# jonnylaw/bayesian_dlms

Measured on AMD Instinct MI355X. Metric: Kalman filter+smooth series*timesteps/sec, higher is better.
Workload: dtype f64

## Files before the change

### bayesian_dlms_amd/csrc/dlm_engine.hip

```cpp
#include "../../include/dlm_engine.h"
#include <cstdlib>
#include "dlm_internal.h"

#include <rccl/rccl.h>

#include <cstdio>
#include <cstring>
#include <set>
#include <string>
#include <vector>

using dlm::KArgs;

struct dlm_engine {
  int device = 0;
  hipStream_t own_stream = nullptr;
  hipStream_t stream = nullptr;
  std::string err;
  const char* variant = "none";
  void* arena = nullptr;
  size_t arena_bytes = 0;
  hipEvent_t ev[3] = {nullptr, nullptr, nullptr};
  bool timed = false;
  dlm::SparseT* sp_dev = nullptr;
// ... 20 lines not shown
    long long f_stride = 0;
    unsigned generic = 0;
    int sparse_k = 0, spb_k = 0, spf_k = 0;
    bool have_spb = false, have_spf = false;
    std::vector<double> g_host, f_host;
  } an;
  bool an_touched = true;
  double* covws = nullptr;
  size_t covws_bytes = 0;
  unsigned char* route = nullptr;
  size_t route_bytes = 0;
  unsigned char* plainbuf = nullptr;
  size_t plainbuf_bytes = 0;
  void* sampws = nullptr;
  size_t sampws_bytes = 0;
  double* zws = nullptr;
  size_t zws_bytes = 0;
  hipStream_t rng_stream = nullptr;
  hipEvent_t rng_ev = nullptr;
  hipStream_t cov_stream = nullptr;
  hipEvent_t cov_ev[2] = {nullptr, nullptr};
  hipEvent_t rng_gate = nullptr;
  hipEvent_t cov_ev2 = nullptr;
  bool cov_busy = false, rng_busy = false;
  unsigned long long* counters = nullptr;
  unsigned long long* model_sum = nullptr;
  int* model_bad = nullptr;
  int* model_bad_dev = nullptr;
  bool model_sum_valid = false;
};

namespace {

int fail(dlm_engine* e, int code, const std::string& msg) {
  if (e) e->err = msg;
  return code;
}

int promise_broken(dlm_engine* e) {
  *e->model_bad = 0;
  e->an.valid = false;
  return fail(e, DLM_ERR_ARG, "DLM_OPT_MODEL_UNCHANGED was set, but F, G or the time grid differ from the model of the previous call (device checksum): the results of this call are invalid -- drop the flag when the model changes");
}

#define HIP_TRY(e, expr)                                                                    \
  do {                                                                                      \
// ... 356 lines not shown
  }
  return DLM_OK;
}
int mark_plain(dlm_engine* e, KArgs& k) {
  k.plain = nullptr;
  if (!(fast_shape_ok(k) && e->sparse_k > 0) || use_lane(k) || !k.y || k.g_index || k.dt || k.f_stride || k.v_tstride || k.w_tstride ||
      (k.flags & DLM_OPT_NO_STEADY)) return DLM_OK;
  if ((size_t)k.N > e->plainbuf_bytes) {
    if (e->plainbuf) { { const int rcd = drain_all(e); if (rcd) return rcd; } HIP_TRY(e, hipFree(e->plainbuf)); e->plainbuf = nullptr; e->plainbuf_bytes = 0; }
    HIP_TRY(e, hipMalloc((void**)&e->plainbuf, (size_t)k.N));
    e->plainbuf_bytes = (size_t)k.N;
  }
  HIP_TRY(e, dlm::launch_sparse16_count_gaps(k, e->plainbuf, e->stream));
  k.plain = e->plainbuf;
  return DLM_OK;
}
int ensure_cov_stream(dlm_engine* e) {
  if (!e->cov_stream) {
    int lo = 0, hi = 0;
    HIP_TRY(e, hipDeviceGetStreamPriorityRange(&lo, &hi));
    HIP_TRY(e, hipStreamCreateWithPriority(&e->cov_stream, hipStreamNonBlocking, hi));
    for (auto& ev : e->cov_ev) HIP_TRY(e, hipEventCreateWithFlags(&ev, hipEventDisableTiming));
    HIP_TRY(e, hipEventCreateWithFlags(&e->cov_ev2, hipEventDisableTiming));
  }
  return DLM_OK;
}
int start_sampler_normals(dlm_engine* e, const KArgs& k, dlm::SampTabs& tb, bool big, hipEvent_t gate);
int start_sampler_tables(dlm_engine* e, const KArgs& k, dlm::SampTabs& tb, bool big, const double* crec = nullptr, int crec_stride = 0, bool defer_normals = false) {
  const size_t need = big ? dlm::wave48_sampler_shared_ws_bytes(k) : dlm::sampler_shared_ws_bytes(k);
  if (need > e->sampws_bytes) {
    if (e->sampws) { { const int rcd = drain_all(e); if (rcd) return rcd; } HIP_TRY(e, hipFree(e->sampws)); e->sampws = nullptr; e->sampws_bytes = 0; }
    HIP_TRY(e, hipMalloc(&e->sampws, need));
    e->sampws_bytes = need;
  }
  int rc = ensure_route(e, (size_t)k.N);
  if (rc || (rc = ensure_cov_stream(e))) return rc;
  if (big) dlm::wave48_sampler_shared_carve(e->sampws, k, tb); else dlm::sampler_shared_carve(e->sampws, k, tb);
  HIP_TRY(e, hipEventRecord(e->cov_ev[0], e->stream));
  e->cov_busy = true;
  HIP_TRY(e, hipStreamWaitEvent(e->cov_stream, e->cov_ev[0], 0));
  tb.zstride = 0; tb.mc4 = nullptr; tb.marked = 0;
  if (big) HIP_TRY(e, dlm::launch_wave48_sampler_shared_tables(k, tb, e->cov_stream, e->cov_ev2));
  else if (crec) HIP_TRY(e, dlm::launch_sampler_shared_tables_from(k, e->sparse_k, e->sp_dev, tb, crec, crec_stride, e->cov_stream));
  else HIP_TRY(e, dlm::launch_sampler_shared_tables(k, e->sparse_k, e->sp_dev, tb, e->cov_stream));
  HIP_TRY(e, hipEventRecord(e->cov_ev[1], e->cov_stream));
  tb.z4 = nullptr;
// ... 24 lines not shown
int start_rts_tables(dlm_engine* e, const KArgs& k, dlm::RtsTabs& tb) {
  const size_t need = dlm::rts_shared_ws_bytes(k);
  if (need > e->sampws_bytes) {
    if (e->sampws) { { const int rcd = drain_all(e); if (rcd) return rcd; } HIP_TRY(e, hipFree(e->sampws)); e->sampws = nullptr; e->sampws_bytes = 0; }
    HIP_TRY(e, hipMalloc(&e->sampws, need));
    e->sampws_bytes = need;
  }
  const size_t cneed = sizeof(double) * dlm::covtabs_doubles(k.d, k.T);
  if (cneed > e->covws_bytes) {
    if (e->covws) { { const int rcd = drain_all(e); if (rcd) return rcd; } HIP_TRY(e, hipFree(e->covws)); e->covws = nullptr; e->covws_bytes = 0; }
    HIP_TRY(e, hipMalloc((void**)&e->covws, cneed));
    e->covws_bytes = cneed;
  }
  int rc = ensure_route(e, (size_t)k.N);
  if (rc || (rc = ensure_cov_stream(e))) return rc;
  dlm::rts_shared_carve(e->sampws, k, tb);
  dlm::CovTabs ctb{};
  dlm::covtabs_carve(e->covws, k.d, k.T, ctb);
  HIP_TRY(e, dlm::launch_rts_shared_mark(k, e->route, tb, e->stream));
  HIP_TRY(e, dlm::launch_rts_shared_cov(k, e->sparse_k, e->sp_dev, tb, ctb, e->stream));
  HIP_TRY(e, hipEventRecord(e->cov_ev[0], e->stream));
  e->cov_busy = true;
  HIP_TRY(e, hipStreamWaitEvent(e->cov_stream, e->cov_ev[0], 0));
  HIP_TRY(e, dlm::launch_rts_shared_tables(k, e->sparse_k, e->sp_dev, tb, e->cov_stream));
  HIP_TRY(e, hipEventRecord(e->cov_ev[1], e->cov_stream));
  return DLM_OK;
}
int ensure_shared(dlm_engine* e, const KArgs& k, dlm::CovTabs& tb, bool with_backward) {
  const size_t need = sizeof(double) * dlm::covtabs_doubles(k.d, k.T);
  if (need > e->covws_bytes) {
    if (e->covws) { { const int rcd = drain_all(e); if (rcd) return rcd; } HIP_TRY(e, hipFree(e->covws)); e->covws = nullptr; e->covws_bytes = 0; }
    HIP_TRY(e, hipMalloc((void**)&e->covws, need));
    e->covws_bytes = need;
  }
  int rc = ensure_route(e, (size_t)k.N);
  if (rc) return rc;
  rc = ensure_side(e, k);
  if (rc) return rc;
  if ((rc = ensure_cov_stream(e))) return rc;
  dlm::covtabs_carve(e->covws, k.d, k.T, tb);
  tb.eq = e->side + 2 * (size_t)k.N * ((size_t)k.T + 1);
  tb.mc = tb.sc = nullptr;
  if (with_backward) {
    const size_t one = 64 * (size_t)((k.N + 3) / 4) * ((size_t)k.T + 1);
    int rc2 = ensure_xplus_bytes(e, sizeof(double) * one);
    if (rc2) return rc2;
    tb.mc = e->xplus;
// ... 127 lines not shown

void dlm_engine_destroy(dlm_engine* e) {
  if (!e) return;
  (void)hipSetDevice(e->device);
  (void)drain_all(e);
  if (e->has_comm) ncclCommDestroy(e->comm);
  if (e->arena) (void)hipFree(e->arena);
  if (e->side) (void)hipFree(e->side);
  if (e->xplus) (void)hipFree(e->xplus);
  if (e->ystar) (void)hipFree(e->ystar);
  if (e->sp_dev) (void)hipFree(e->sp_dev);
  if (e->fws) (void)hipFree(e->fws);
  if (e->spb_dev) (void)hipFree(e->spb_dev);
  if (e->spf_dev) (void)hipFree(e->spf_dev);
  if (e->covws) (void)hipFree(e->covws);
  if (e->route) (void)hipFree(e->route);
  if (e->plainbuf) (void)hipFree(e->plainbuf);
  if (e->sampws) (void)hipFree(e->sampws);
  if (e->zws) (void)hipFree(e->zws);
  if (e->rng_ev) (void)hipEventDestroy(e->rng_ev);
  if (e->rng_stream) (void)hipStreamDestroy(e->rng_stream);
  for (auto& ev : e->cov_ev) if (ev) (void)hipEventDestroy(ev);
  if (e->cov_ev2) (void)hipEventDestroy(e->cov_ev2);
  if (e->rng_gate) (void)hipEventDestroy(e->rng_gate);
  if (e->cov_stream) (void)hipStreamDestroy(e->cov_stream);
  if (e->counters) (void)hipFree(e->counters);
  if (e->model_sum) (void)hipFree(e->model_sum);
  if (e->model_bad) (void)hipHostFree(e->model_bad);
  for (void* b : e->buffers) (void)hipFree(b);
  if (e->order_ev) (void)hipEventDestroy(e->order_ev);
  for (auto& ev : e->ev) if (ev) (void)hipEventDestroy(ev);
  if (e->own_stream) (void)hipStreamDestroy(e->own_stream);
  delete e;
}

const char* dlm_last_error(const dlm_engine* e) { return e ? e->err.c_str() : "null engine"; }
const char* dlm_last_variant(const dlm_engine* e) { return e ? e->variant : "none"; }

int dlm_engine_set_stream(dlm_engine* e, void* hip_stream) {
  if (!e) return DLM_ERR_ARG;
  hipStream_t next = hip_stream ? (hipStream_t)hip_stream : e->own_stream;
  if (next != e->stream) {
    HIP_TRY(e, hipSetDevice(e->device));
    { const int rcd = drain_all(e); if (rcd) return rcd; }
    e->stream = next;
  }
// ... 388 lines not shown
                          (q1 ? !fused_fast : fast_smoother_ok(e, k)) && dlm::rts_shared_eligible(k, !q1);
  if (!filt) {
    k.packed |= (fast_smoother_ok(e, k) && e->sparse_k > 0 && !use_lane(k) && !rts_shared) ? 1 : 0;
    if ((rc = ensure_fws(e, (k.packed & 1) ? N * (T + 1) * (size_t)dlm::packed_rec_bytes((int)d) : N * (T + 1) * rec * sizeof(double)))) return rc;
    k.filt = e->fws;
  }
  if ((rc = mark(e, 0))) return rc;
  dlm::RtsTabs rtb{};
  if (rts_shared && (rc = start_rts_tables(e, k, rtb))) return rc;
  if (rts_shared && (k.flags & DLM_OPT_TEST_FAIL_AFTER_TABLES))
    return fail(e, DLM_ERR_UNSUPPORTED, "DLM_OPT_TEST_FAIL_AFTER_TABLES");
  if ((rc = mark_plain(e, k))) return rc;
  if (filt && fast_smoother_ok(e, k) && use_shared_cov(e, k)) {
    dlm::CovTabs tb;
    if ((rc = run_shared_filter(e, k, tb, true))) return rc;
    if ((rc = mark(e, 1))) return rc;
    k.filt_in = k.filt;
    if ((rc = run_shared_smoother(e, k, tb))) return rc;
    if ((rc = mark(e, 2))) return rc;
    return st.finish(opts->flags & DLM_OPT_ASYNC);
  }
  if ((rc = run_filter(e, k, fused_fast))) return rc;
  if (rts_shared) {
    HIP_TRY(e, hipStreamWaitEvent(e->stream, e->cov_ev[1], 0));
    e->cov_busy = false;
  }
  if ((rc = mark(e, 1))) return rc;
  k.filt_in = k.filt;
  if (rts_shared) {
    k.route = e->route; k.route_take = 0;
    e->variant = "sparse16-rts-shared";
    HIP_TRY(e, dlm::launch_rts_shared_means(k, e->sparse_k, e->sp_dev, rtb, q1, e->stream));
    if (!q1) {
      KArgs kg = k;
      kg.route_take = 1;
      HIP_TRY(e, dlm::launch_sparse16_smoother(kg, e->sparse_k, e->sp_dev, e->side, e->stream));
    }
  } else if ((rc = run_smoother(e, k, fused_fast))) return rc;
  if ((rc = mark(e, 2))) return rc;
  return st.finish(opts->flags & DLM_OPT_ASYNC);
}

static int sampler_common(dlm_engine* e, const dlm_model_desc* model, const dlm_params_desc* params,
                          const double* y, const double* z, const dlm_options* opts,
                          const double* filt_in, double* filt_ws, double* theta, double* cond,
                          double* stats, int32_t* status, bool forward) {
  int rc = check_common(e, model, params, opts);
  if (rc) return rc;
  AuxScope aux(e);
  const bool norec = forward && !filt_ws;
  if (forward && !y) return fail(e, DLM_ERR_ARG, "y is required");
  if (!forward && !filt_in) return fail(e, DLM_ERR_ARG, "filter records are required");
  if (stats && !y) return fail(e, DLM_ERR_ARG, "sufficient statistics need y");
  const size_t d = model->d, p = model->p, T = model->T, N = model->N, rec = d + d * d;
  KArgs k{};
// ... 277 lines not shown
```

### bayesian_dlms_amd/csrc/dlm_internal.h

```cpp
#pragma once
#include <hip/hip_runtime.h>
#include <stdint.h>

namespace dlm {

struct KArgs {
  int d, p, T, N;
  const double* F; long long f_stride;
  const double* G; int n_g; const int* g_index; const double* dt;
  const double* V; long long v_stride;
  const double* W; long long w_stride;
  long long v_tstride, w_tstride;
  const double* m0; long long m0_stride;
  const double* C0; long long c0_stride;
  const double* y;
  const double* z;
  const double* filt_in;
  double* filt;
  double* prior;
  double* fq;
  double* smooth;
  double* theta;
  double* cond;
  double* stats;
// ... 77 lines not shown
  int marked;
  double* ktab;
  int* settle;
};
bool sampler_shared_model_ok(const KArgs& a);
bool sampler_shared_eligible(const KArgs& a);
size_t sampler_shared_ws_bytes(const KArgs& a);
void sampler_shared_carve(void* ws, const KArgs& a, SampTabs& tb);
hipError_t launch_sampler_shared_tables(const KArgs& a, int K, const SparseT* tabs_dev, const SampTabs& tb, hipStream_t s);
hipError_t launch_sampler_shared_tables_from(const KArgs& a, int K, const SparseT* tabs_dev, SampTabs tb, const double* crec, int stride, hipStream_t s);
size_t sampler_shared_normals_bytes(const KArgs& a);
hipError_t launch_sampler_shared_normals(const KArgs& a, double* z4, hipStream_t s);
hipError_t launch_sampler_shared_draw(const KArgs& a, int K, const SparseT* tabs_dev, const SampTabs& tb, hipStream_t s);

struct RtsTabs {
  double* jrows;
  double* srec;
  unsigned char* need;
  int* status;
  const double* crec;
  int crec_stride;
  int* gaps;
  int* skip;
};
bool rts_shared_eligible(const KArgs& a, bool textbook);
size_t rts_shared_ws_bytes(const KArgs& a);
void rts_shared_carve(void* ws, const KArgs& a, RtsTabs& tb);
hipError_t launch_rts_shared_cov(const KArgs& a, int K, const SparseT* tabs_dev, RtsTabs& tb, const CovTabs& ctb, hipStream_t s);
hipError_t launch_rts_shared_tables(const KArgs& a, int K, const SparseT* tabs_dev, const RtsTabs& tb, hipStream_t s);
hipError_t launch_rts_shared_mark(const KArgs& a, unsigned char* route, const RtsTabs& tb, hipStream_t s);
hipError_t launch_rts_shared_means(const KArgs& a, int K, const SparseT* tabs_dev, const RtsTabs& tb, bool own_rts, hipStream_t s);

bool wave48_sampler_shared_model_ok(const KArgs& a);
bool wave48_sampler_shared_eligible(const KArgs& a);
size_t wave48_sampler_shared_ws_bytes(const KArgs& a);
void wave48_sampler_shared_carve(void* ws, const KArgs& a, SampTabs& tb);
hipError_t launch_wave48_sampler_shared_tables(const KArgs& a, const SampTabs& tb, hipStream_t s, hipEvent_t after_filter = nullptr);
hipError_t launch_wave48_sampler_shared_draw(const KArgs& a, const SampTabs& tb, hipStream_t s);
size_t wave48_ktab_doubles(const KArgs& a);
hipError_t launch_wave48_steady_filter(const KArgs& a, const double* ktab, const int* settle, hipStream_t s);
hipError_t launch_wave48_mark_gaps(const KArgs& a, unsigned char* route, hipStream_t s);
size_t wave48_sampler_shared_normals_bytes(const KArgs& a);
hipError_t launch_wave48_sampler_shared_normals(const KArgs& a, double* z, hipStream_t s);

struct SparseBig { int K; int pad; int idx[48][4]; double val[48][4]; };
int sparse48_analyse(const double* G_host, int d, SparseBig* rows, SparseBig* cols);
struct SparseF { int K; int pad; int cidx[32][4]; double cval[32][4]; int ridx[48][4]; double rval[48][4]; };
int sparsef_analyse(const double* F_host, int d, int p, SparseF* out);
bool tiled_supported(const KArgs& a);
hipError_t launch_tiled_filter(const KArgs& a, double* innov, hipStream_t s);
hipError_t launch_tiled_smoother(const KArgs& a, const double* innov, hipStream_t s);
bool wave48_small_shape(const KArgs& a);
bool wave48_small_ok(const KArgs& a);
bool wave48_filter_supported(const KArgs& a);
// ... 145 lines not shown
```

### bayesian_dlms_amd/csrc/dlm_sampler16.hip

```cpp
#include "dlm_internal.h"
#include "../../include/dlm_engine.h"

namespace dlm {
namespace s16 {

typedef double d4 __attribute__((ext_vector_type(4)));
typedef unsigned u2 __attribute__((ext_vector_type(2)));
constexpr int IL = 17;
constexpr int IMG = 16 * IL;
constexpr int OOB = 0x7ffffff0;

__device__ __forceinline__ void wave_sync() {
  __builtin_amdgcn_fence(__ATOMIC_RELEASE, "wavefront");
  __builtin_amdgcn_wave_barrier();
  __builtin_amdgcn_fence(__ATOMIC_ACQUIRE, "wavefront");
}
__device__ __forceinline__ double sum_g(double v) {
  unsigned lo = (unsigned)__double2loint(v), hi = (unsigned)__double2hiint(v);
  u2 l = __builtin_amdgcn_permlane16_swap(lo, lo, false, false);
  u2 h = __builtin_amdgcn_permlane16_swap(hi, hi, false, false);
  v = __hiloint2double((int)h[0], (int)l[0]) + __hiloint2double((int)h[1], (int)l[1]);
  lo = (unsigned)__double2loint(v); hi = (unsigned)__double2hiint(v);
  l = __builtin_amdgcn_permlane32_swap(lo, lo, false, false);
  h = __builtin_amdgcn_permlane32_swap(hi, hi, false, false);
// ... 720 lines not shown
  int ridx[K];
  double rval[K];
  int gcur = -1;
  auto load_tables = [&](int gi) {
#pragma unroll
    for (int s = 0; s < K; ++s) { ridx[s] = sp[2 * gi].idx[c][s]; rval[s] = vc ? sp[2 * gi].val[c][s] : 0.0; }
    gcur = gi;
  };
  const double* W0 = a.W + (size_t)n * a.w_stride;
  d4 Wt;
  bool va[4];
  int offC[4];
#pragma unroll
  for (int r = 0; r < 4; ++r) {
    const int i = 4 * r + g;
    va[r] = i < d && vc;
    offC[r] = va[r] ? (d + i + c * d) * 8 : OOB;
    Wt[r] = va[r] ? W0[i + c * d] : 0.0;
  }
  const int offM = (vc && g == 0) ? c * 8 : OOB;
  const int rstr = (EXP && tb.crec) ? tb.crec_stride : recb;
  const __amdgpu_buffer_rsrc_t rin = (EXP && tb.crec) ? mk_rsrc(tb.crec, (size_t)(T + 1) * rstr) : mk_rsrc(a.filt_in + (size_t)n * (T + 1) * rec, (size_t)(T + 1) * recb);
  const __amdgpu_buffer_rsrc_t rout = mk_rsrc(a.smooth + (size_t)n * (T + 1) * rec, (size_t)(T + 1) * recb);
  int st = 0;
  d4 S, Rinv = {0.0, 0.0, 0.0, 0.0};
  bool warm = false;
  {
#pragma unroll
    for (int r = 0; r < 4; ++r) { S[r] = bld(rin, offC[r], T * rstr); bst(rout, offC[r], T * recb, S[r]); }
    const double mc = bld(rin, vc ? c * 8 : OOB, T * rstr);
    bst(rout, offM, T * recb, mc);
    if (g == 0) sv[c] = mc;
    wave_sync();
    if constexpr (EXP) { if (lane == 0) tb.need[T] = 0; }
  }
  d4 Cp = {0.0, 0.0, 0.0, 0.0}, JTs = Cp, Js = Cp, Rs = Cp;
  bool have = false;
  int gprev = -1;
  double dtprev = 0.0, cmaxp = 0.0;
  d4 nC;
  double nm;
  {
    const int tp = T > 0 ? T - 1 : 0;
#pragma unroll
    for (int r = 0; r < 4; ++r) nC[r] = bld(rin, offC[r], tp * rstr);
    nm = bld(rin, vc ? c * 8 : OOB, tp * rstr);
  }
  double scol = 0.0;
  for (int t = T - 1; t >= 0; --t) {
    const double dt = a.dt ? a.dt[t] : 1.0;
    const int gi = a.g_index ? a.g_index[t] : 0;
    if (gi != gcur) load_tables(gi);
    const d4 C = nC;
    const double mc = nm;
    {
      const int tp = t > 0 ? t - 1 : 0;
#pragma unroll
      for (int r = 0; r < 4; ++r) nC[r] = bld(rin, offC[r], tp * rstr);
      nm = bld(rin, vc ? c * 8 : OOB, tp * rstr);
    }
    if (a.w_tstride) {
#pragma unroll
      for (int r = 0; r < 4; ++r) Wt[r] = va[r] ? (W0 + (size_t)t * a.w_tstride)[4 * r + g + c * d] : 0.0;
    }
    if (!EXP && g == 0) mv[c] = mc;
    bool reuse = false;
    if (have && gi == gprev && dt == dtprev && !a.w_tstride) {
      bool moved = false;
#pragma unroll
      for (int r = 0; r < 4; ++r) moved |= !(fabs(C[r] - Cp[r]) <= DLM_SETTLE_TOL * cmaxp);
      reuse = __ballot(moved) == 0ull;
    }
// ... 63 lines not shown
            const bool any_big = __ballot(big) != 0ull, any_far = __ballot(far) != 0ull;
            if (any_far && any_big) break;
            if (!any_big) done = true;
            const d4 D = mm(Rinv, E, d);
#pragma unroll
            for (int r = 0; r < 4; ++r) Rinv[r] += D[r];
            const d4 Xt = transposed(Rinv, img, g, c);
#pragma unroll
            for (int r = 0; r < 4; ++r) Rinv[r] = 0.5 * (Rinv[r] + Xt[r]);
          }
        }
        if (!done && direct_inverse(R, Rinv, d, img, inv, lane, g, c)) st |= DLM_ST_NOT_PD;
        warm = true;
      }
      JT = mm(Rinv, GC, d);
      J = mm(GC, Rinv, d);
      if constexpr (EXP) {
        double* row = tb.jrows + (size_t)t * RJ_ROW + c * RJ_ENT;
        if (vc) {
#pragma unroll
          for (int r = 0; r < 4; ++r) row[4 * r + g] = JT[r];
        }
        if (lane == 0) tb.need[t] = 1;
      }
      Cp = C; JTs = JT; Js = J; Rs = R; have = true; gprev = gi; dtprev = dt;
      {
        double mx = fmax(fmax(fabs(C[0]), fabs(C[1])), fmax(fabs(C[2]), fabs(C[3])));
        for (int o_ = 32; o_ > 0; o_ >>= 1) mx = fmax(mx, __shfl_xor(mx, o_));
        cmaxp = mx;
      }
    }
    if constexpr (!EXP) {
      if (g == 0) uv[c] = vc ? sv[c] - a1 : 0.0;
      wave_sync();
      scol = mc + matTvec(JT, uv, g);
    }
    d4 X;
#pragma unroll
    for (int r = 0; r < 4; ++r) X[r] = R[r] - S[r];
    const d4 Y = mm(X, JT, d);
    const d4 JXJ = compat ? mm(Y, J, d) : mm(JT, Y, d);
#pragma unroll
    for (int r = 0; r < 4; ++r) { S[r] = va[r] ? C[r] - JXJ[r] : 0.0; bst(rout, offC[r], t * recb, S[r]); }
    bst(rout, offM, t * recb, scol);
    if constexpr (!EXP) {
      wave_sync();
      if (g == 0) sv[c] = vc ? scol : 0.0;
      wave_sync();
    }
  }
  bool bad = vc && g == 0 && !isfinite(scol);
#pragma unroll
  for (int r = 0; r < 4; ++r) bad |= va[r] && !isfinite(S[r]);
  if (__ballot(bad) != 0ull) st |= DLM_ST_NONFINITE;
  if (a.status && lane == 0 && st) atomicOr(&a.status[n], st);
}

#ifndef DLM_RTS_STORE_AUX
#define DLM_RTS_STORE_AUX 2
#endif
__device__ __forceinline__ void bst128(__amdgpu_buffer_rsrc_t r, int voff, int soff, d2 x) {
  typedef unsigned u4 __attribute__((ext_vector_type(4)));
  const u4 v = {(unsigned)__double2loint(x[0]), (unsigned)__double2hiint(x[0]), (unsigned)__double2loint(x[1]), (unsigned)__double2hiint(x[1])};
  __builtin_amdgcn_raw_buffer_store_b128(v, r, voff, soff, DLM_RTS_STORE_AUX);
}
__device__ __forceinline__ d2 lds_read128v(unsigned addr) {
  d2 v;
  asm volatile("ds_read_b128 %0, %1" : "=v"(v) : "v"(addr) : "memory");
  return v;
}
template <int NP>
__device__ __forceinline__ void lds_wait_np(d2 (&pc)[NP]) {
  static_assert(NP == 2 || NP == 4 || NP == 6 || NP == 8, "pieces");
  if constexpr (NP == 2) asm volatile("s_waitcnt lgkmcnt(0)" : "+v"(pc[0]), "+v"(pc[1])::"memory");
  else if constexpr (NP == 4) asm volatile("s_waitcnt lgkmcnt(0)" : "+v"(pc[0]), "+v"(pc[1]), "+v"(pc[2]), "+v"(pc[3])::"memory");
  else if constexpr (NP == 6) asm volatile("s_waitcnt lgkmcnt(0)" : "+v"(pc[0]), "+v"(pc[1]), "+v"(pc[2]), "+v"(pc[3]), "+v"(pc[4]), "+v"(pc[5])::"memory");
  else asm volatile("s_waitcnt lgkmcnt(0)" : "+v"(pc[0]), "+v"(pc[1]), "+v"(pc[2]), "+v"(pc[3]), "+v"(pc[4]), "+v"(pc[5]), "+v"(pc[6]), "+v"(pc[7])::"memory");
}

template <int K, int NP, int NRS, int NRJ>
__global__ __launch_bounds__(64, 3) void k_mean_rts16(KArgs a, const SparseT* __restrict__ sp, RtsTabs tb) {
  __shared__ __attribute__((aligned(16))) double lds[2 * 64 + 2 * (RS_SLOT / 8) + 2 * RJ_ROW + SF_AHEAD * 64];
  const int lane = threadIdx.x, j = lane >> 4, c = lane & 15;
  const int n0 = 4 * blockIdx.x;
  if (n0 >= a.N) return;
  const int nser = a.N - n0 < 4 ? a.N - n0 : 4;
  const bool have = j < nser;
  const int n = have ? n0 + j : n0;
  const bool dead = !have || a.route[n] != 0;
  unsigned deadmask = 0;
#pragma unroll
  for (int q = 0; q < 4; ++q) deadmask |= (__builtin_amdgcn_readlane((int)dead, 16 * q) & 1) << q;
  if (a.counters && lane == 0) {
    const int routed = __builtin_popcount(deadmask & ((1u << nser) - 1u));
    if (nser - routed) atomicAdd(&a.counters[2], (unsigned long long)(nser - routed));
    if (routed) atomicAdd(&a.counters[3], (unsigned long long)routed);
  }
  if (deadmask == 0xfu) return;
  double* vU = lds;
  double* vH = vU + 64;
  char* ring = (char*)(vH + 64);
  const int d = a.d, T = a.T, rec = d + d * d, recb = rec * 8;
  const bool vc = c < d;
  int idx[K];
  double val[K];
#pragma unroll
  for (int s = 0; s < K; ++s) { idx[s] = (16 * j + sp[0].idx[c][s]) * 8; val[s] = vc ? sp[0].val[c][s] : 0.0; }
  const size_t sbytes = (size_t)(T + 1) * recb;
  const i4 rmean = rsrc_words((const char*)a.filt_in + (size_t)n0 * sbytes, (unsigned)((size_t)nser * sbytes));
  const i4 rjt = rsrc_words(tb.jrows, (unsigned)((size_t)(T + 1) * RJ_ROW * 8));
  const i4 rst = rsrc_words(tb.srec, (unsigned)sbytes);
  const __amdgpu_buffer_rsrc_t rout = mk_rsrc((char*)a.smooth + (size_t)n0 * sbytes, (size_t)nser * sbytes);
  const int mvoff = (lane < 32 && (lane >> 3) < nser) ? (int)((size_t)(lane >> 3) * sbytes) + (lane & 7) * 16 : OOB;
  const unsigned sring_lds = lds_addr_of(ring), jring_lds = sring_lds + 2 * RS_SLOT, mring_lds = jring_lds + 2 * (RJ_ROW * 8);
  const unsigned vH_lds = lds_addr_of(vH);
  const int npc = rec / 2;
  const int nj16 = d * (RJ_ENT / 2);
  auto dma_means = [&](unsigned lds_addr, int soff) {
    lds_addr = (unsigned)__builtin_amdgcn_readfirstlane((int)lds_addr);
    soff = __builtin_amdgcn_readfirstlane(soff);
    if (lane < 32)
      asm volatile("s_mov_b32 m0, %0\n\ts_nop 0\n\tbuffer_load_dwordx4 %1, %2, %3 offen lds" ::"s"(lds_addr), "v"(mvoff), "s"(rmean), "s"(soff) : "memory");
  };
  unsigned psrc[NP];
  int pdst[NP];
// ... 5 lines not shown
  }
  const unsigned ptd = (unsigned)(c * 8);
  const unsigned char* need = tb.need;

  double Jc[16];
#pragma unroll
  for (int k = 0; k < 16; ++k) Jc[k] = 0.0;
  auto read_J = [&](unsigned slot) {
    const unsigned base = slot + (vc ? c : 0) * (RJ_ENT * 8);
    d2 q[8];
    q[0] = lds_read128<0>(base); q[1] = lds_read128<16>(base); q[2] = lds_read128<32>(base); q[3] = lds_read128<48>(base);
    q[4] = lds_read128<64>(base); q[5] = lds_read128<80>(base); q[6] = lds_read128<96>(base); q[7] = lds_read128<112>(base);
    asm volatile("s_waitcnt lgkmcnt(0)" : "+v"(q[0]), "+v"(q[1]), "+v"(q[2]), "+v"(q[3]), "+v"(q[4]), "+v"(q[5]), "+v"(q[6]), "+v"(q[7])::"memory");
#pragma unroll
    for (int k = 0; k < 8; ++k) { Jc[2 * k] = q[k][0]; Jc[2 * k + 1] = q[k][1]; }
  };
  auto emit = [&](int t, unsigned sslot, unsigned jslot, unsigned mslot, bool nd2) {
    d2 pc[NP];
#pragma unroll
    for (int k = 0; k < NP; ++k) pc[k] = lds_read128v((psrc[k] & 0x80000000u) ? vH_lds + (psrc[k] & 0x7fffffffu) : sslot + psrc[k]);
    lds_wait_np<NP>(pc);
    dma_means(mslot, (t > SF_AHEAD ? t - SF_AHEAD : 0) * recb);
    if (nd2) dma_row<NRJ>(rjt, jslot, (t - 2) * (RJ_ROW * 8), lane, nj16);
    dma_row<NRS>(rst, sslot, (t > 1 ? t - 2 : 0) * recb, lane, npc);
    const int so = t * recb;
#pragma unroll
    for (int k = 0; k < NP; ++k) bst128(rout, pdst[k], so, pc[k]);
  };

  for (int k = 0; k < SF_AHEAD; ++k) { const int tk = T - k > 0 ? T - k : 0; dma_means(mring_lds + ((T - k) & (SF_AHEAD - 1)) * 512, tk * recb); }
  dma_row<NRS>(rst, sring_lds + (T & 1) * RS_SLOT, T * recb, lane, npc);
  dma_row<NRS>(rst, sring_lds + ((T - 1) & 1) * RS_SLOT, (T - 1) * recb, lane, npc);
  unsigned long long nmask = 0;
  auto need_of = [&](int s_) -> bool {
    if (s_ < 0) return false;
    if (s_ == T || (s_ & 63) == 63) { const int b = (s_ & ~63) + lane; nmask = __ballot(b <= T && need[b] != 0); }
    return ((nmask >> (s_ & 63)) & 1ull) != 0;
  };
  bool nd0 = need_of(T), nd1 = need_of(T - 1), nd2 = need_of(T - 2);
  (void)nd0;
  if (nd1) dma_row<NRJ>(rjt, jring_lds + ((T - 1) & 1) * (RJ_ROW * 8), (T - 1) * (RJ_ROW * 8), lane, nj16);
  double sc;
  {
    vm_wait<0>();
    wave_sync();
    const unsigned sslot = sring_lds + (T & 1) * RS_SLOT, mslot = mring_lds + (T & (SF_AHEAD - 1)) * 512;
    double mr = lds_read64<0>(mslot + lane * 8), td = lds_read64<0>(sslot + ptd);
    asm volatile("s_waitcnt lgkmcnt(0)" : "+v"(mr), "+v"(td)::"memory");
    sc = vc ? mr : 0.0;
    vH[lane] = vc ? mr : td;
    wave_sync();
    emit(T, sslot, jring_lds + (T & 1) * (RJ_ROW * 8), mslot, nd2);
  }
  for (int t = T - 1; t >= 0; --t) {
    nd0 = nd1; nd1 = nd2; nd2 = need_of(t - 2);
    if (nd1) vm_wait<2 * NP + 1 + NRS + NRJ>(); else vm_wait<2 * NP + 1 + NRS>();
    const unsigned sslot = sring_lds + (t & 1) * RS_SLOT, jslot = jring_lds + (t & 1) * (RJ_ROW * 8), mslot = mring_lds + (t & (SF_AHEAD - 1)) * 512;
    double mr = lds_read64<0>(mslot + lane * 8), td = lds_read64<0>(sslot + ptd);
    double mg[K];
#pragma unroll
    for (int s = 0; s < K; ++s) mg[s] = lds_read64<0>(mslot + idx[s]);
    if constexpr (K == 1) asm volatile("s_waitcnt lgkmcnt(0)" : "+v"(mr), "+v"(td), "+v"(mg[0])::"memory");
    else if constexpr (K == 2) asm volatile("s_waitcnt lgkmcnt(0)" : "+v"(mr), "+v"(td), "+v"(mg[0]), "+v"(mg[1])::"memory");
    else if constexpr (K == 3) asm volatile("s_waitcnt lgkmcnt(0)" : "+v"(mr), "+v"(td), "+v"(mg[0]), "+v"(mg[1]), "+v"(mg[2])::"memory");
    else asm volatile("s_waitcnt lgkmcnt(0)" : "+v"(mr), "+v"(td), "+v"(mg[0]), "+v"(mg[1]), "+v"(mg[2]), "+v"(mg[3])::"memory");
    if (nd0) read_J(jslot);
    const double mc = vc ? mr : 0.0;
    double a1 = 0.0;
#pragma unroll
    for (int s = 0; s < K; ++s) a1 = fma(vc ? mg[s] : 0.0, val[s], a1);
    vU[lane] = vc ? sc - a1 : 0.0;
    wave_sync();
    double ch[4] = {0.0, 0.0, 0.0, 0.0};
#pragma unroll
    for (int r = 0; r < 4; ++r)
#pragma unroll
      for (int g = 0; g < 4; ++g) ch[g] = fma(Jc[4 * r + g], vU[16 * j + 4 * r + g], ch[g]);
    const double scol = mc + ((ch[0] + ch[1]) + (ch[2] + ch[3]));
    vH[lane] = vc ? scol : td;
    wave_sync();
    emit(t, sslot, jslot, mslot, nd2);
    sc = vc ? scol : 0.0;
  }
  vm_wait<0>();
  const int stz = tb.status[0];
  const unsigned long long badl = __ballot(!dead && vc && !isfinite(sc));
  if (!dead && c == 0) {
    const int sj = stz | (((badl >> (16 * j)) & 0xffffull) ? DLM_ST_NONFINITE : 0);
    if (a.status && sj) atomicOr(&a.status[n], sj);
  }
}

}

template <class Tab>
static hipError_t launch_sampler_t(const KArgs& a, int K, const Tab* tabs_dev, hipStream_t s) {
  switch (K) {
    case 1: hipLaunchKernelGGL((s16::k_sampler_sp16<1, Tab>), dim3(a.N), dim3(64), 0, s, a, tabs_dev, SampTabs{}); break;
    case 2: hipLaunchKernelGGL((s16::k_sampler_sp16<2, Tab>), dim3(a.N), dim3(64), 0, s, a, tabs_dev, SampTabs{}); break;
    case 3: hipLaunchKernelGGL((s16::k_sampler_sp16<3, Tab>), dim3(a.N), dim3(64), 0, s, a, tabs_dev, SampTabs{}); break;
    case 4: hipLaunchKernelGGL((s16::k_sampler_sp16<4, Tab>), dim3(a.N), dim3(64), 0, s, a, tabs_dev, SampTabs{}); break;
    default: return hipErrorInvalidValue;
  }
  return hipGetLastError();
}
hipError_t launch_sparse16_sampler(const KArgs& a, int K, const SparseT* tabs_dev, hipStream_t s) { return launch_sampler_t(a, K, tabs_dev, s); }

// ... 125 lines not shown
    case 1: DLM_MS(1); break;
    case 2: DLM_MS(2); break;
    case 3: DLM_MS(3); break;
    case 4: DLM_MS(4); break;
    default: return hipErrorInvalidValue;
  }
#undef DLM_MS
  if (err != hipSuccess) return err;
  KArgs kg = a;
  kg.route_take = 1;
  return launch_sampler_t(kg, K, tabs_dev, s);
}

#ifndef DLM_RTS_SHARED_MIN
#define DLM_RTS_SHARED_MIN 2048
#endif
#ifndef DLM_RTS_SHARED_MIN_TEXTBOOK
#define DLM_RTS_SHARED_MIN_TEXTBOOK 6144
#endif
bool rts_shared_eligible(const KArgs& a, bool textbook) {
  return sampler_shared_model_ok(a) && a.y && !(a.flags & (DLM_OPT_FORCE_GENERIC | DLM_OPT_SMOOTHER_PER_SERIES | DLM_OPT_NO_STEADY)) &&
         (a.N >= (textbook ? DLM_RTS_SHARED_MIN_TEXTBOOK : DLM_RTS_SHARED_MIN) || (a.flags & DLM_OPT_NO_SMALL_BATCH));
}
size_t rts_shared_ws_bytes(const KArgs& a) {
  const size_t n1 = (size_t)a.T + 1, rec = (size_t)a.d + (size_t)a.d * a.d;
  return up64(n1 * s16::RJ_ROW * 8) + up64(n1 * rec * 8) + up64(n1) + 64;
}
void rts_shared_carve(void* ws, const KArgs& a, RtsTabs& tb) {
  const size_t n1 = (size_t)a.T + 1, rec = (size_t)a.d + (size_t)a.d * a.d;
  char* p = (char*)ws;
  tb.jrows = (double*)p; p += up64(n1 * s16::RJ_ROW * 8);
  tb.srec = (double*)p;  p += up64(n1 * rec * 8);
  tb.need = (unsigned char*)p; p += up64(n1);
  tb.status = (int*)p; tb.gaps = tb.status + 8; tb.skip = tb.status + 9;
  tb.crec = nullptr; tb.crec_stride = 0;
}
hipError_t launch_rts_shared_cov(const KArgs& a, int K, const SparseT* tabs_dev, RtsTabs& tb, const CovTabs& ctb, hipStream_t s) {
  KArgs kc = a;
  kc.smooth = nullptr; kc.filt = nullptr; kc.stats = nullptr; kc.theta = nullptr; kc.z = nullptr;
  tb.crec = ctb.ftab; tb.crec_stride = ctb.frow;
  CovTabs cs = ctb;
  cs.skip = tb.skip;
  return launch_sparse16_cov_filter(kc, K, tabs_dev, cs, s);
}
template <int TAG, class F>
static size_t whole_cu_lds(F kernel) {
  auto ask = [&]() -> size_t {
    hipFuncAttributes at;
    if (hipFuncGetAttributes(&at, (const void*)kernel) != hipSuccess) { (void)hipGetLastError(); return 0; }
    const size_t whole = 160 * 1024;
    if (at.sharedSizeBytes >= whole) return 0;
    const size_t dyn = whole - at.sharedSizeBytes;
    if (hipFuncSetAttribute((const void*)kernel, hipFuncAttributeMaxDynamicSharedMemorySize, (int)dyn) != hipSuccess) { (void)hipGetLastError(); return 0; }
    return dyn;
  };
  static const size_t dyn = ask();
  return dyn;
}
hipError_t launch_rts_shared_tables(const KArgs& a, int K, const SparseT* tabs_dev, const RtsTabs& tb, hipStream_t s) {
  KArgs kp = a;
  kp.N = 1; kp.y = nullptr; kp.m0_stride = 0; kp.filt_in = nullptr; kp.filt = nullptr; kp.smooth = tb.srec; kp.status = tb.status; kp.stats = nullptr; kp.loglik = nullptr;
  kp.prior = nullptr; kp.fq = nullptr; kp.route = nullptr; kp.counters = nullptr; kp.theta = nullptr; kp.z = nullptr; kp.series_offset = 0; kp.plain = nullptr;
  switch (K) {
    case 1: hipLaunchKernelGGL((s16::k_smoother_rts16<1, SparseT, true>), dim3(1), dim3(64), whole_cu_lds<1>(s16::k_smoother_rts16<1, SparseT, true>), s, kp, tabs_dev, tb); break;
    case 2: hipLaunchKernelGGL((s16::k_smoother_rts16<2, SparseT, true>), dim3(1), dim3(64), whole_cu_lds<2>(s16::k_smoother_rts16<2, SparseT, true>), s, kp, tabs_dev, tb); break;
    case 3: hipLaunchKernelGGL((s16::k_smoother_rts16<3, SparseT, true>), dim3(1), dim3(64), whole_cu_lds<3>(s16::k_smoother_rts16<3, SparseT, true>), s, kp, tabs_dev, tb); break;
    case 4: hipLaunchKernelGGL((s16::k_smoother_rts16<4, SparseT, true>), dim3(1), dim3(64), whole_cu_lds<4>(s16::k_smoother_rts16<4, SparseT, true>), s, kp, tabs_dev, tb); break;
    default: return hipErrorInvalidValue;
  }
  return hipGetLastError();
}
template <int K>
static hipError_t launch_mean_rts(const KArgs& a, const SparseT* sp, const RtsTabs& tb, hipStream_t s) {
  const dim3 grid((a.N + 3) / 4), blk(64);
  const int d = a.d;
  if (d <= 7) hipLaunchKernelGGL((s16::k_mean_rts16<K, 2, 1, 1>), grid, blk, 0, s, a, sp, tb);
  else if (d <= 10) hipLaunchKernelGGL((s16::k_mean_rts16<K, 4, 1, 2>), grid, blk, 0, s, a, sp, tb);
  else if (d <= 13) hipLaunchKernelGGL((s16::k_mean_rts16<K, 6, 2, 2>), grid, blk, 0, s, a, sp, tb);
  else if (d == 14) hipLaunchKernelGGL((s16::k_mean_rts16<K, 8, 2, 2>), grid, blk, 0, s, a, sp, tb);
  else hipLaunchKernelGGL((s16::k_mean_rts16<K, 8, 2, 3>), grid, blk, 0, s, a, sp, tb);
  return hipGetLastError();
}
hipError_t launch_rts_shared_mark(const KArgs& a, unsigned char* route, const RtsTabs& tb, hipStream_t s) {
  if (!route || !a.y) return hipErrorInvalidValue;
  hipError_t err = hipMemsetAsync(tb.status, 0, 16 * sizeof(int), s);
  if (err != hipSuccess) return err;
  hipLaunchKernelGGL(s16::k_mark_gaps, dim3((a.N + 3) / 4), dim3(256), 0, s, a.y, a.N, a.T, route, tb.gaps);
  if ((err = hipGetLastError()) != hipSuccess) return err;
  hipLaunchKernelGGL(s16::k_rts_decide, dim3((a.N + 255) / 256), dim3(256), 0, s, route, a.N, (const int*)tb.gaps, tb.skip);
  return hipGetLastError();
}
hipError_t launch_rts_shared_means(const KArgs& a, int K, const SparseT* tabs_dev, const RtsTabs& tb, bool own_rts, hipStream_t s) {
  if (!a.route || !a.y) return hipErrorInvalidValue;
  hipError_t err;
  KArgs km = a;
  km.route_take = 0;
  switch (K) {
    case 1: err = launch_mean_rts<1>(km, tabs_dev, tb, s); break;
    case 2: err = launch_mean_rts<2>(km, tabs_dev, tb, s); break;
    case 3: err = launch_mean_rts<3>(km, tabs_dev, tb, s); break;
    case 4: err = launch_mean_rts<4>(km, tabs_dev, tb, s); break;
    default: return hipErrorInvalidValue;
  }
  if (err != hipSuccess || !own_rts) return err;
  KArgs kg = a;
  kg.route_take = 1;
  return launch_rts_t(kg, K, tabs_dev, s);
}

hipError_t launch_sparse16_rts(const KArgs& a, int K, const SparseT* tabs_dev, hipStream_t s) { return launch_rts_t(a, K, tabs_dev, s); }
hipError_t launch_small_mv_rts(const KArgs& a, hipStream_t s) { return launch_rts_t(a, a.spb_k, a.spb, s); }
hipError_t launch_small_mv_sampler(const KArgs& a, hipStream_t s) { return launch_sampler_t(a, a.spb_k, a.spb, s); }

}
```

Baseline: 1.250 billion.

## Split shared RTS table backward pass into two blocks to overlap with mean smoothing

The shared RTS covariance/gain table kernel on the side stream is split at a time index (a third of T by default, for T of at least 256) into two launches. The main stream waits only for the first block (late timesteps) before starting the per-series mean smoother over those timesteps, then waits for the second block before finishing the rest. Recursion state is checkpointed to a device buffer between launches. The aim is to overlap the serial table recursion with the parallel mean pass, at the cost of extra launches, state save/restore and carry buffers.

```diff
diff --git a/bayesian_dlms_amd/csrc/dlm_engine.hip b/bayesian_dlms_amd/csrc/dlm_engine.hip
--- a/bayesian_dlms_amd/csrc/dlm_engine.hip
+++ b/bayesian_dlms_amd/csrc/dlm_engine.hip
@@ -66,6 +66,7 @@
   hipEvent_t cov_ev[2] = {nullptr, nullptr};
   hipEvent_t rng_gate = nullptr;
   hipEvent_t cov_ev2 = nullptr;
+  hipEvent_t cov_blk = nullptr;
   bool cov_busy = false, rng_busy = false;
   unsigned long long* counters = nullptr;
   unsigned long long* model_sum = nullptr;
@@ -468,6 +469,7 @@
     HIP_TRY(e, hipStreamCreateWithPriority(&e->cov_stream, hipStreamNonBlocking, hi));
     for (auto& ev : e->cov_ev) HIP_TRY(e, hipEventCreateWithFlags(&ev, hipEventDisableTiming));
     HIP_TRY(e, hipEventCreateWithFlags(&e->cov_ev2, hipEventDisableTiming));
+    HIP_TRY(e, hipEventCreateWithFlags(&e->cov_blk, hipEventDisableTiming));
   }
   return DLM_OK;
 }
@@ -538,7 +540,11 @@
   HIP_TRY(e, hipEventRecord(e->cov_ev[0], e->stream));
   e->cov_busy = true;
   HIP_TRY(e, hipStreamWaitEvent(e->cov_stream, e->cov_ev[0], 0));
-  HIP_TRY(e, dlm::launch_rts_shared_tables(k, e->sparse_k, e->sp_dev, tb, e->cov_stream));
+  HIP_TRY(e, dlm::launch_rts_shared_tables(k, e->sparse_k, e->sp_dev, tb, 0, e->cov_stream));
+  if (tb.split) {
+    HIP_TRY(e, hipEventRecord(e->cov_blk, e->cov_stream));
+    HIP_TRY(e, dlm::launch_rts_shared_tables(k, e->sparse_k, e->sp_dev, tb, 1, e->cov_stream));
+  }
   HIP_TRY(e, hipEventRecord(e->cov_ev[1], e->cov_stream));
   return DLM_OK;
 }
@@ -712,6 +718,7 @@
   if (e->rng_stream) (void)hipStreamDestroy(e->rng_stream);
   for (auto& ev : e->cov_ev) if (ev) (void)hipEventDestroy(ev);
   if (e->cov_ev2) (void)hipEventDestroy(e->cov_ev2);
+  if (e->cov_blk) (void)hipEventDestroy(e->cov_blk);
   if (e->rng_gate) (void)hipEventDestroy(e->rng_gate);
   if (e->cov_stream) (void)hipStreamDestroy(e->cov_stream);
   if (e->counters) (void)hipFree(e->counters);
@@ -1146,15 +1153,20 @@
   }
   if ((rc = run_filter(e, k, fused_fast))) return rc;
   if (rts_shared) {
-    HIP_TRY(e, hipStreamWaitEvent(e->stream, e->cov_ev[1], 0));
-    e->cov_busy = false;
+    HIP_TRY(e, hipStreamWaitEvent(e->stream, rtb.split ? e->cov_blk : e->cov_ev[1], 0));
+    if (!rtb.split) e->cov_busy = false;
   }
   if ((rc = mark(e, 1))) return rc;
   k.filt_in = k.filt;
   if (rts_shared) {
     k.route = e->route; k.route_take = 0;
     e->variant = "sparse16-rts-shared";
-    HIP_TRY(e, dlm::launch_rts_shared_means(k, e->sparse_k, e->sp_dev, rtb, q1, e->stream));
+    if (rtb.split) {
+      HIP_TRY(e, dlm::launch_rts_shared_means(k, e->sparse_k, e->sp_dev, rtb, 0, false, e->stream));
+      HIP_TRY(e, hipStreamWaitEvent(e->stream, e->cov_ev[1], 0));
+      e->cov_busy = false;
+    }
+    HIP_TRY(e, dlm::launch_rts_shared_means(k, e->sparse_k, e->sp_dev, rtb, rtb.split ? 1 : 0, q1, e->stream));
     if (!q1) {
       KArgs kg = k;
       kg.route_take = 1;
diff --git a/bayesian_dlms_amd/csrc/dlm_internal.h b/bayesian_dlms_amd/csrc/dlm_internal.h
--- a/bayesian_dlms_amd/csrc/dlm_internal.h
+++ b/bayesian_dlms_amd/csrc/dlm_internal.h
@@ -123,14 +123,21 @@
   int crec_stride;
   int* gaps;
   int* skip;
-};
+  int split;
+  int block;
+  double* state;
+  double* sk;
+};
+constexpr int RTS_ST_DOUBLES = 26;
+constexpr int RTS_ST_INTS = 5;
+int rts_shared_split(const KArgs& a);
 bool rts_shared_eligible(const KArgs& a, bool textbook);
 size_t rts_shared_ws_bytes(const KArgs& a);
 void rts_shared_carve(void* ws, const KArgs& a, RtsTabs& tb);
 hipError_t launch_rts_shared_cov(const KArgs& a, int K, const SparseT* tabs_dev, RtsTabs& tb, const CovTabs& ctb, hipStream_t s);
-hipError_t launch_rts_shared_tables(const KArgs& a, int K, const SparseT* tabs_dev, const RtsTabs& tb, hipStream_t s);
+hipError_t launch_rts_shared_tables(const KArgs& a, int K, const SparseT* tabs_dev, const RtsTabs& tb, int block, hipStream_t s);
 hipError_t launch_rts_shared_mark(const KArgs& a, unsigned char* route, const RtsTabs& tb, hipStream_t s);
-hipError_t launch_rts_shared_means(const KArgs& a, int K, const SparseT* tabs_dev, const RtsTabs& tb, bool own_rts, hipStream_t s);
+hipError_t launch_rts_shared_means(const KArgs& a, int K, const SparseT* tabs_dev, const RtsTabs& tb, int block, bool own_rts, hipStream_t s);
 
 bool wave48_sampler_shared_model_ok(const KArgs& a);
 bool wave48_sampler_shared_eligible(const KArgs& a);
diff --git a/bayesian_dlms_amd/csrc/dlm_sampler16.hip b/bayesian_dlms_amd/csrc/dlm_sampler16.hip
--- a/bayesian_dlms_amd/csrc/dlm_sampler16.hip
+++ b/bayesian_dlms_amd/csrc/dlm_sampler16.hip
@@ -766,10 +766,17 @@
   const int rstr = (EXP && tb.crec) ? tb.crec_stride : recb;
   const __amdgpu_buffer_rsrc_t rin = (EXP && tb.crec) ? mk_rsrc(tb.crec, (size_t)(T + 1) * rstr) : mk_rsrc(a.filt_in + (size_t)n * (T + 1) * rec, (size_t)(T + 1) * recb);
   const __amdgpu_buffer_rsrc_t rout = mk_rsrc(a.smooth + (size_t)n * (T + 1) * rec, (size_t)(T + 1) * recb);
+  const int t_top = (EXP && tb.split && tb.block) ? tb.split : T;
+  const int t_end = (EXP && tb.split && !tb.block) ? tb.split : 0;
   int st = 0;
   d4 S, Rinv = {0.0, 0.0, 0.0, 0.0};
   bool warm = false;
-  {
+  d4 Cp = {0.0, 0.0, 0.0, 0.0}, JTs = Cp, Js = Cp, Rs = Cp;
+  bool have = false;
+  int gprev = -1;
+  double dtprev = 0.0, cmaxp = 0.0;
+  int jlast = T;
+  if (t_top == T) {
 #pragma unroll
     for (int r = 0; r < 4; ++r) { S[r] = bld(rin, offC[r], T * rstr); bst(rout, offC[r], T * recb, S[r]); }
     const double mc = bld(rin, vc ? c * 8 : OOB, T * rstr);
@@ -777,21 +784,27 @@
     if (g == 0) sv[c] = mc;
     wave_sync();
     if constexpr (EXP) { if (lane == 0) tb.need[T] = 0; }
-  }
-  d4 Cp = {0.0, 0.0, 0.0, 0.0}, JTs = Cp, Js = Cp, Rs = Cp;
-  bool have = false;
-  int gprev = -1;
-  double dtprev = 0.0, cmaxp = 0.0;
+  } else if constexpr (EXP) {
+    const double* sd = tb.state;
+    const int* si = (const int*)(tb.state + RTS_ST_DOUBLES * 64);
+#pragma unroll
+    for (int r = 0; r < 4; ++r) {
+      S[r] = sd[(0 + r) * 64 + lane]; Rinv[r] = sd[(4 + r) * 64 + lane]; Cp[r] = sd[(8 + r) * 64 + lane];
+      JTs[r] = sd[(12 + r) * 64 + lane]; Js[r] = sd[(16 + r) * 64 + lane]; Rs[r] = sd[(20 + r) * 64 + lane];
+    }
+    cmaxp = sd[24 * 64 + lane]; dtprev = sd[25 * 64 + lane];
+    warm = si[0 * 64 + lane] != 0; have = si[1 * 64 + lane] != 0; gprev = si[2 * 64 + lane]; st = si[3 * 64 + lane]; jlast = si[4 * 64 + lane];
+  }
   d4 nC;
   double nm;
   {
-    const int tp = T > 0 ? T - 1 : 0;
+    const int tp = t_top > 0 ? t_top - 1 : 0;
 #pragma unroll
     for (int r = 0; r < 4; ++r) nC[r] = bld(rin, offC[r], tp * rstr);
     nm = bld(rin, vc ? c * 8 : OOB, tp * rstr);
   }
   double scol = 0.0;
-  for (int t = T - 1; t >= 0; --t) {
+  for (int t = t_top - 1; t >= t_end; --t) {
     const double dt = a.dt ? a.dt[t] : 1.0;
     const int gi = a.g_index ? a.g_index[t] : 0;
     if (gi != gcur) load_tables(gi);
@@ -901,6 +914,7 @@
           for (int r = 0; r < 4; ++r) row[4 * r + g] = JT[r];
         }
         if (lane == 0) tb.need[t] = 1;
+        jlast = t;
       }
       Cp = C; JTs = JT; Js = J; Rs = R; have = true; gprev = gi; dtprev = dt;
       {
@@ -928,6 +942,20 @@
       wave_sync();
     }
   }
+  if constexpr (EXP) {
+    if (t_end > 0) {
+      double* sd = tb.state;
+      int* si = (int*)(tb.state + RTS_ST_DOUBLES * 64);
+#pragma unroll
+      for (int r = 0; r < 4; ++r) {
+        sd[(0 + r) * 64 + lane] = S[r]; sd[(4 + r) * 64 + lane] = Rinv[r]; sd[(8 + r) * 64 + lane] = Cp[r];
+        sd[(12 + r) * 64 + lane] = JTs[r]; sd[(16 + r) * 64 + lane] = Js[r]; sd[(20 + r) * 64 + lane] = Rs[r];
+      }
+      sd[24 * 64 + lane] = cmaxp; sd[25 * 64 + lane] = dtprev;
+      si[0 * 64 + lane] = warm ? 1 : 0; si[1 * 64 + lane] = have ? 1 : 0; si[2 * 64 + lane] = gprev; si[3 * 64 + lane] = st; si[4 * 64 + lane] = jlast;
+      return;
+    }
+  }
   bool bad = vc && g == 0 && !isfinite(scol);
 #pragma unroll
   for (int r = 0; r < 4; ++r) bad |= va[r] && !isfinite(S[r]);
@@ -964,13 +992,16 @@
   const int n0 = 4 * blockIdx.x;
   if (n0 >= a.N) return;
   const int nser = a.N - n0 < 4 ? a.N - n0 : 4;
+  const int T = a.T;
+  const int t_top = (tb.split && tb.block) ? tb.split : T;
+  const int t_end = (tb.split && !tb.block) ? tb.split : 0;
   const bool have = j < nser;
   const int n = have ? n0 + j : n0;
   const bool dead = !have || a.route[n] != 0;
   unsigned deadmask = 0;
 #pragma unroll
   for (int q = 0; q < 4; ++q) deadmask |= (__builtin_amdgcn_readlane((int)dead, 16 * q) & 1) << q;
-  if (a.counters && lane == 0) {
+  if (a.counters && lane == 0 && t_top == T) {
     const int routed = __builtin_popcount(deadmask & ((1u << nser) - 1u));
     if (nser - routed) atomicAdd(&a.counters[2], (unsigned long long)(nser - routed));
     if (routed) atomicAdd(&a.counters[3], (unsigned long long)routed);
@@ -979,7 +1010,7 @@
   double* vU = lds;
   double* vH = vU + 64;
   char* ring = (char*)(vH + 64);
-  const int d = a.d, T = a.T, rec = d + d * d, recb = rec * 8;
+  const int d = a.d, rec = d + d * d, recb = rec * 8;
   const bool vc = c < d;
   int idx[K];
   double val[K];
@@ -1031,26 +1062,27 @@
     lds_wait_np<NP>(pc);
     dma_means(mslot, (t > SF_AHEAD ? t - SF_AHEAD : 0) * recb);
     if (nd2) dma_row<NRJ>(rjt, jslot, (t - 2) * (RJ_ROW * 8), lane, nj16);
-    dma_row<NRS>(rst, sslot, (t > 1 ? t - 2 : 0) * recb, lane, npc);
+    dma_row<NRS>(rst, sslot, (t - 2 > t_end ? t - 2 : t_end) * recb, lane, npc);
     const int so = t * recb;
 #pragma unroll
     for (int k = 0; k < NP; ++k) bst128(rout, pdst[k], so, pc[k]);
   };
 
-  for (int k = 0; k < SF_AHEAD; ++k) { const int tk = T - k > 0 ? T - k : 0; dma_means(mring_lds + ((T - k) & (SF_AHEAD - 1)) * 512, tk * recb); }
-  dma_row<NRS>(rst, sring_lds + (T & 1) * RS_SLOT, T * recb, lane, npc);
-  dma_row<NRS>(rst, sring_lds + ((T - 1) & 1) * RS_SLOT, (T - 1) * recb, lane, npc);
   unsigned long long nmask = 0;
   auto need_of = [&](int s_) -> bool {
-    if (s_ < 0) return false;
-    if (s_ == T || (s_ & 63) == 63) { const int b = (s_ & ~63) + lane; nmask = __ballot(b <= T && need[b] != 0); }
+    if (s_ < t_end) return false;
+    if (s_ == t_top || (s_ & 63) == 63) { const int b = (s_ & ~63) + lane; nmask = __ballot(b <= T && b >= t_end && need[b] != 0); }
     return ((nmask >> (s_ & 63)) & 1ull) != 0;
   };
-  bool nd0 = need_of(T), nd1 = need_of(T - 1), nd2 = need_of(T - 2);
-  (void)nd0;
-  if (nd1) dma_row<NRJ>(rjt, jring_lds + ((T - 1) & 1) * (RJ_ROW * 8), (T - 1) * (RJ_ROW * 8), lane, nj16);
   double sc;
-  {
+  bool nd0, nd1, nd2;
+  if (t_top == T) {
+    for (int k = 0; k < SF_AHEAD; ++k) { const int tk = T - k > 0 ? T - k : 0; dma_means(mring_lds + ((T - k) & (SF_AHEAD - 1)) * 512, tk * recb); }
+    dma_row<NRS>(rst, sring_lds + (T & 1) * RS_SLOT, T * recb, lane, npc);
+    dma_row<NRS>(rst, sring_lds + ((T - 1) & 1) * RS_SLOT, (T - 1) * recb, lane, npc);
+    nd0 = need_of(T); nd1 = need_of(T - 1); nd2 = need_of(T - 2);
+    (void)nd0;
+    if (nd1) dma_row<NRJ>(rjt, jring_lds + ((T - 1) & 1) * (RJ_ROW * 8), (T - 1) * (RJ_ROW * 8), lane, nj16);
     vm_wait<0>();
     wave_sync();
     const unsigned sslot = sring_lds + (T & 1) * RS_SLOT, mslot = mring_lds + (T & (SF_AHEAD - 1)) * 512;
@@ -1060,8 +1092,24 @@
     vH[lane] = vc ? mr : td;
     wave_sync();
     emit(T, sslot, jring_lds + (T & 1) * (RJ_ROW * 8), mslot, nd2);
-  }
-  for (int t = T - 1; t >= 0; --t) {
+  } else {
+    sc = tb.sk[(size_t)blockIdx.x * 64 + lane];
+    const int jl = __builtin_amdgcn_readfirstlane(((const int*)(tb.state + RTS_ST_DOUBLES * 64))[4 * 64]);
+    const unsigned jk = jring_lds + (t_top & 1) * (RJ_ROW * 8);
+    dma_row<NRJ>(rjt, jk, jl * (RJ_ROW * 8), lane, nj16);
+    vm_wait<0>();
+    wave_sync();
+    read_J(jk);
+    for (int k = 1; k <= SF_AHEAD; ++k) if (t_top - k >= 0) dma_means(mring_lds + ((t_top - k) & (SF_AHEAD - 1)) * 512, (t_top - k) * recb);
+    for (int k = 1; k <= 2; ++k) if (t_top - k >= 0) dma_row<NRS>(rst, sring_lds + ((t_top - k) & 1) * RS_SLOT, (t_top - k) * recb, lane, npc);
+    nd0 = need_of(t_top); nd1 = need_of(t_top - 1); nd2 = need_of(t_top - 2);
+    (void)nd0;
+    if (nd1) dma_row<NRJ>(rjt, jring_lds + ((t_top - 1) & 1) * (RJ_ROW * 8), (t_top - 1) * (RJ_ROW * 8), lane, nj16);
+    if (nd2) dma_row<NRJ>(rjt, jring_lds + ((t_top - 2) & 1) * (RJ_ROW * 8), (t_top - 2) * (RJ_ROW * 8), lane, nj16);
+    vm_wait<0>();
+    wave_sync();
+  }
+  for (int t = t_top - 1; t >= t_end; --t) {
     nd0 = nd1; nd1 = nd2; nd2 = need_of(t - 2);
     if (nd1) vm_wait<2 * NP + 1 + NRS + NRJ>(); else vm_wait<2 * NP + 1 + NRS>();
     const unsigned sslot = sring_lds + (t & 1) * RS_SLOT, jslot = jring_lds + (t & 1) * (RJ_ROW * 8), mslot = mring_lds + (t & (SF_AHEAD - 1)) * 512;
@@ -1092,6 +1140,7 @@
     sc = vc ? scol : 0.0;
   }
   vm_wait<0>();
+  if (t_end > 0) { tb.sk[(size_t)blockIdx.x * 64 + lane] = sc; return; }
   const int stz = tb.status[0];
   const unsigned long long badl = __ballot(!dead && vc && !isfinite(sc));
   if (!dead && c == 0) {
@@ -1263,9 +1312,24 @@
   return sampler_shared_model_ok(a) && a.y && !(a.flags & (DLM_OPT_FORCE_GENERIC | DLM_OPT_SMOOTHER_PER_SERIES | DLM_OPT_NO_STEADY)) &&
          (a.N >= (textbook ? DLM_RTS_SHARED_MIN_TEXTBOOK : DLM_RTS_SHARED_MIN) || (a.flags & DLM_OPT_NO_SMALL_BATCH));
 }
+#ifndef DLM_RTS_SPLIT_PCT
+#define DLM_RTS_SPLIT_PCT 33
+#endif
+#ifndef DLM_RTS_SPLIT_MIN_T
+#define DLM_RTS_SPLIT_MIN_T 256
+#endif
+#ifndef DLM_RTS_BLOCK1_WHOLE_CU
+#define DLM_RTS_BLOCK1_WHOLE_CU 0
+#endif
+int rts_shared_split(const KArgs& a) {
+  if (a.T < DLM_RTS_SPLIT_MIN_T || DLM_RTS_SPLIT_PCT <= 0) return 0;
+  const int k = (int)((long long)a.T * DLM_RTS_SPLIT_PCT / 100);
+  return (k >= 2 && k <= a.T - 2) ? k : 0;
+}
 size_t rts_shared_ws_bytes(const KArgs& a) {
   const size_t n1 = (size_t)a.T + 1, rec = (size_t)a.d + (size_t)a.d * a.d;
-  return up64(n1 * s16::RJ_ROW * 8) + up64(n1 * rec * 8) + up64(n1) + 64;
+  return up64(n1 * s16::RJ_ROW * 8) + up64(n1 * rec * 8) + up64(n1) + 64 +
+         up64(64 * (RTS_ST_DOUBLES * 8 + RTS_ST_INTS * 4)) + up64((size_t)((a.N + 3) / 4) * 64 * 8);
 }
 void rts_shared_carve(void* ws, const KArgs& a, RtsTabs& tb) {
   const size_t n1 = (size_t)a.T + 1, rec = (size_t)a.d + (size_t)a.d * a.d;
@@ -1273,8 +1337,12 @@
   tb.jrows = (double*)p; p += up64(n1 * s16::RJ_ROW * 8);
   tb.srec = (double*)p;  p += up64(n1 * rec * 8);
   tb.need = (unsigned char*)p; p += up64(n1);
-  tb.status = (int*)p; tb.gaps = tb.status + 8; tb.skip = tb.status + 9;
+  tb.status = (int*)p; tb.gaps = tb.status + 8; tb.skip = tb.status + 9; p += 64;
   tb.crec = nullptr; tb.crec_stride = 0;
+  tb.state = (double*)p; p += up64(64 * (RTS_ST_DOUBLES * 8 + RTS_ST_INTS * 4));
+  tb.sk = (double*)p;
+  tb.split = rts_shared_split(a);
+  tb.block = 0;
 }
 hipError_t launch_rts_shared_cov(const KArgs& a, int K, const SparseT* tabs_dev, RtsTabs& tb, const CovTabs& ctb, hipStream_t s) {
   KArgs kc = a;
@@ -1298,15 +1366,18 @@
   static const size_t dyn = ask();
   return dyn;
 }
-hipError_t launch_rts_shared_tables(const KArgs& a, int K, const SparseT* tabs_dev, const RtsTabs& tb, hipStream_t s) {
+hipError_t launch_rts_shared_tables(const KArgs& a, int K, const SparseT* tabs_dev, const RtsTabs& tb0, int block, hipStream_t s) {
+  RtsTabs tb = tb0;
+  tb.block = block;
+  const bool whole = block == 0 || DLM_RTS_BLOCK1_WHOLE_CU;
   KArgs kp = a;
   kp.N = 1; kp.y = nullptr; kp.m0_stride = 0; kp.filt_in = nullptr; kp.filt = nullptr; kp.smooth = tb.srec; kp.status = tb.status; kp.stats = nullptr; kp.loglik = nullptr;
   kp.prior = nullptr; kp.fq = nullptr; kp.route = nullptr; kp.counters = nullptr; kp.theta = nullptr; kp.z = nullptr; kp.series_offset = 0; kp.plain = nullptr;
   switch (K) {
-    case 1: hipLaunchKernelGGL((s16::k_smoother_rts16<1, SparseT, true>), dim3(1), dim3(64), whole_cu_lds<1>(s16::k_smoother_rts16<1, SparseT, true>), s, kp, tabs_dev, tb); break;
-    case 2: hipLaunchKernelGGL((s16::k_smoother_rts16<2, SparseT, true>), dim3(1), dim3(64), whole_cu_lds<2>(s16::k_smoother_rts16<2, SparseT, true>), s, kp, tabs_dev, tb); break;
-    case 3: hipLaunchKernelGGL((s16::k_smoother_rts16<3, SparseT, true>), dim3(1), dim3(64), whole_cu_lds<3>(s16::k_smoother_rts16<3, SparseT, true>), s, kp, tabs_dev, tb); break;
-    case 4: hipLaunchKernelGGL((s16::k_smoother_rts16<4, SparseT, true>), dim3(1), dim3(64), whole_cu_lds<4>(s16::k_smoother_rts16<4, SparseT, true>), s, kp, tabs_dev, tb); break;
+    case 1: hipLaunchKernelGGL((s16::k_smoother_rts16<1, SparseT, true>), dim3(1), dim3(64), whole ? whole_cu_lds<1>(s16::k_smoother_rts16<1, SparseT, true>) : 0, s, kp, tabs_dev, tb); break;
+    case 2: hipLaunchKernelGGL((s16::k_smoother_rts16<2, SparseT, true>), dim3(1), dim3(64), whole ? whole_cu_lds<2>(s16::k_smoother_rts16<2, SparseT, true>) : 0, s, kp, tabs_dev, tb); break;
+    case 3: hipLaunchKernelGGL((s16::k_smoother_rts16<3, SparseT, true>), dim3(1), dim3(64), whole ? whole_cu_lds<3>(s16::k_smoother_rts16<3, SparseT, true>) : 0, s, kp, tabs_dev, tb); break;
+    case 4: hipLaunchKernelGGL((s16::k_smoother_rts16<4, SparseT, true>), dim3(1), dim3(64), whole ? whole_cu_lds<4>(s16::k_smoother_rts16<4, SparseT, true>) : 0, s, kp, tabs_dev, tb); break;
     default: return hipErrorInvalidValue;
   }
   return hipGetLastError();
@@ -1331,8 +1402,10 @@
   hipLaunchKernelGGL(s16::k_rts_decide, dim3((a.N + 255) / 256), dim3(256), 0, s, route, a.N, (const int*)tb.gaps, tb.skip);
   return hipGetLastError();
 }
-hipError_t launch_rts_shared_means(const KArgs& a, int K, const SparseT* tabs_dev, const RtsTabs& tb, bool own_rts, hipStream_t s) {
+hipError_t launch_rts_shared_means(const KArgs& a, int K, const SparseT* tabs_dev, const RtsTabs& tb0, int block, bool own_rts, hipStream_t s) {
   if (!a.route || !a.y) return hipErrorInvalidValue;
+  RtsTabs tb = tb0;
+  tb.block = block;
   hipError_t err;
   KArgs km = a;
   km.route_take = 0;
```

New measurement: 1.255 billion, median of 6. Within noise of the previous version (+0.4%).
